# caskcsg/lightretriever

Hardware: AMD Instinct MI355X
Metric: docs embedded/sec (llama3.2-1b dims, seq_len=512, bf16) [+ queries/sec@top-100 over 1000000-doc index in `search`] (higher is better)
Workload: dtype bf16

## Files before the change

include/lrx.h:

```cpp
#ifndef LRX_H
#define LRX_H

#include <stddef.h>
#include <stdint.h>

#ifdef __cplusplus
extern "C" {
#endif

#define LRX_ABI_VERSION 8

enum {
  LRX_OK = 0,
  LRX_ERR_INVALID = -1,
  LRX_ERR_HIP = -2,
  LRX_ERR_WORKSPACE = -3,
};

int lrx_abi_version(void);
const char* lrx_last_error(void);

typedef struct lrx_encoder_config {
  int32_t vocab_size;
  int32_t hidden_size;
// ... 125 lines not shown
                       int32_t capacity, int32_t* ids_out, int32_t* weights_out, int32_t* counts_out, void* stream);

int lrx_sparse_csr_count(const float* reps, int32_t n_rows, int32_t vocab_size, int64_t row_stride, int32_t quantization_factor,
                         int32_t empty_marker, int32_t* counts_out, void* stream);
int lrx_sparse_csr_fill(const float* reps, int32_t n_rows, int32_t vocab_size, int64_t row_stride, int32_t quantization_factor,
                        int32_t empty_marker, const int64_t* row_off, int32_t* terms_out, int32_t* weights_out, void* stream);

int lrx_hit_contributions(const double* scores, const int64_t* ids, int32_t n_queries, int32_t k, int64_t row_stride,
                          int32_t method, double param0, double param1, double* contrib_out, int64_t contrib_row_stride,
                          void* stream);
int lrx_hit_union(const int64_t* ids, const double* contrib, int32_t n_queries, int32_t n_entries, int64_t row_stride,
                  double* scores_out, int64_t* ids_out, int32_t* counts_out, void* stream);

int lrx_gemm_bf16_nt_fused(const void* A, const void* B, void* C, const void* bias, const void* resid, int32_t M, int32_t N,
                           int32_t K, int32_t epilogue, const float* rscale, float* ss_part, void* stream);
int lrx_gemm_qkv_rope_fused(const void* A, const void* Wqkv, void* C, const void* bias, const int32_t* positions,
                            const float* cos, const float* sin, int32_t M, int32_t K, int32_t num_q_heads,
                            int32_t num_kv_heads, int32_t head_dim, const float* rscale, void* stream);
int lrx_gemm_qkv_rope_slice(const void* A, const void* Wqkv, void* C, const void* bias, const int32_t* positions,
                            const float* cos, const float* sin, int32_t M, int32_t K, int32_t num_q_heads,
                            int32_t num_kv_heads, int32_t head_dim, const float* rscale, int32_t head0, int32_t n_heads, void* stream);
int lrx_gemm_bf16_nt_resid32(const void* A, const void* B, float* x32, void* a16_out, const void* gamma, int32_t M, int32_t N,
                             int32_t K, float* ss_part, void* stream);
int lrx_embed_stream32(const void* table, const int32_t* ids, int32_t n_tokens, int32_t hidden, int32_t vocab, const void* gamma,
                       float* x32, void* a16, float* rscale_out, float eps, void* stream);
int lrx_rmsnorm_f32(const float* x, const void* w, void* y, int32_t rows, int32_t hidden, float eps, void* stream);
int lrx_row_rscale(const void* x, int32_t rows, int32_t hidden_size, float eps, float* rscale_out, void* stream);
int lrx_finalize_rscale(const float* ss_part, int32_t n_parts, int32_t rows, int32_t hidden_size, float eps, float* rscale_out,
                        void* stream);

int lrx_gather_last_rows(const void* src, const int32_t* cu_seqlens, int32_t n_seqs, int32_t width, void* dst, void* stream);
int lrx_scatter_last_rows(const void* src, const int32_t* cu_seqlens, int32_t n_seqs, int32_t width, void* dst, int64_t dst_row_stride,
                          void* stream);

int lrx_pool_norm(const void* hidden, const void* final_norm_w, const int32_t* cu_seqlens, int32_t n_seqs,
                  int32_t hidden_size, float eps, float* out, int64_t out_row_stride, int32_t out_dim,
                  int32_t normalize, void* stream);
int lrx_pool_norm_shard(const void* hidden, const void* final_norm_w, const int32_t* cu_seqlens, int32_t n_seqs,
                        int32_t hidden_size, float eps, float* out, int64_t out_row_stride, int32_t out_dim,
                        int32_t normalize, void* shadow_out, int64_t shadow_row0, float* row_bounds, int32_t hidden_f32, void* stream);

int lrx_pool_norm_mode(const void* hidden, const void* final_norm_w, const int32_t* cu_seqlens, int32_t n_seqs,
                       int32_t hidden_size, float eps, int32_t pooling, float* out, int64_t out_row_stride, int32_t out_dim,
                       int32_t normalize, void* shadow_out, int64_t shadow_row0, float* row_bounds, int32_t hidden_f32, void* stream);

int lrx_embedding_bag_mean(const float* table, int32_t vocab, int32_t hidden, const int64_t* ids, int64_t n_ids,
// ... 129 lines not shown
```

lightretriever_amd/_lib.py:

```python
import ctypes as C
import os

HERE = os.path.dirname(os.path.abspath(__file__))
LIB_PATH = os.environ.get("LRX_LIB_DEV_VARIANT") or os.path.join(HERE, "liblrx.so")
LRX_PROF_CLASSES = 8
ABI_VERSION = 8
SEARCH_FILTER_AUTO, SEARCH_FILTER_MATRIX, SEARCH_FILTER_SCORE_FREE, SEARCH_FILTER_SCORE_FREE_NO_GEMM = 0, 1, 2, 3
SEARCH_FUSED_ALWAYS, SEARCH_FUSED_NEVER = 4, 8
SEARCH_REFINE_ROWS_ALWAYS, SEARCH_REFINE_ROWS_NEVER = 16, 32
BINARY_SELECT_ONLY = 1
PROF_CLASS_NAMES = ["gemm_store", "gemm_resid", "gemm_swiglu", "attention", "rmsnorm", "rope", "other", "gemm_maxagg"]


class LrxError(RuntimeError):
    pass


class EncoderConfigC(C.Structure):
    _fields_ = [("vocab_size", C.c_int32), ("hidden_size", C.c_int32), ("num_layers", C.c_int32), ("num_q_heads", C.c_int32),
                ("num_kv_heads", C.c_int32), ("head_dim", C.c_int32), ("intermediate_size", C.c_int32), ("rms_eps", C.c_float),
                ("qkv_bias", C.c_int32), ("max_positions", C.c_int32), ("norm_folded", C.c_int32), ("precise_stream", C.c_int32)]


class LayerWeightsC(C.Structure):
# ... 60 lines not shown
    "lrx_pq_ip_search": (_I32, [_P, _I64, _P, _I32, _I32, _P, _I32, _I32, _I64, _P, _P, _P, _P, _SZ, _I32, _P]),
    "lrx_pq_encode": (_I32, [_P, _I64, _I64, _P, _I32, _I32, _P, _I64, _P]),
    "lrx_pq_decode_rows": (_I32, [_P, _I64, _I64, _P, _I32, _I32, _P, _I64, _P]),
    "lrx_pq_lut": (_I32, [_P, _I32, _P, _I32, _I32, _P, _P]),
    "lrx_binary_workspace_bytes": (_SZ, [_I64, _I32, _I32, _I32]),
    "lrx_binary_hamming_search": (_I32, [_P, _I64, _I32, _P, _I32, _F, _P, _I32, _I64, _P, _P, _P, _P, _SZ, _I32, _P]),
    "lrx_binary_ip_search": (_I32, [_P, _I64, _I32, _P, _I32, _F, _P, _I32, _I32, _I64, _P, _P, _P, _P, _SZ, _I32, _P]),
    "lrx_binary_pack_rows": (_I32, [_P, _I64, _I64, _I32, _F, _P, _P, _I64, _P]),
    "lrx_binary_store_rows": (_I32, [_P, _I64, _I64, _I32, _P, _I64, _P]),
    "lrx_binary_decode_rows": (_I32, [_P, _I64, _I64, _I32, _P, _I64, _P]),
    "lrx_sq8_ip_workspace_bytes": (_SZ, [_I64, _I32, _I32, _I32]),
    "lrx_sq8_ip_chunk_queries": (_I32, [_I64, _I32, _I32, _I32]),
    "lrx_sq8_ip_search": (_I32, [_P, _I64, _P, _I32, _I32, _P, _I32, _I32, _I64, _P, _P, _P, _P, _SZ, _I32, _P]),
    "lrx_sq8_train_minmax": (_I32, [_P, _I64, _I64, _I32, _P, _P]),
    "lrx_sq8_encode": (_I32, [_P, _I64, _I64, _P, _I32, _I32, _P, _I64, _P]),
    "lrx_sq8_decode_rows": (_I32, [_P, _I64, _I64, _P, _I32, _I32, _P, _I64, _P]),
    "lrx_linear_transform": (_I32, [_P, _I64, _I64, _P, _P, _I32, _I32, _P, _I64, _P]),
    "lrx_impact_workspace_bytes": (_SZ, [_I64, _I32, _I32]),
    "lrx_impact_chunk_queries": (_I32, [_I64, _I32, _I32]),
    "lrx_impact_search": (_I32, [_P, _P, _I32, _I64, _P, _P, _P, _I32, _I32, _I64, _P, _P, _P, _P, _SZ, _I32, _P]),
    "lrx_shard_commit_rows": (_I32, [_P, _I64, _I64, _I32, _P, _I64, _P, _P]),
    "lrx_pool_norm_shard": (_I32, [_P, _P, _P, _I32, _I32, _F, _P, _I64, _I32, _I32, _P, _I64, _P, _I32, _P]),
    "lrx_gemm_bf16_nt_resid32": (_I32, [_P, _P, _P, _P, _P, _I32, _I32, _I32, _P, _P]),
    "lrx_embed_stream32": (_I32, [_P, _P, _I32, _I32, _I32, _P, _P, _P, _P, _F, _P]),
    "lrx_rmsnorm_f32": (_I32, [_P, _P, _P, _I32, _I32, _F, _P]),
    "lrx_gemm_bf16_nt_fused": (_I32, [_P, _P, _P, _P, _P, _I32, _I32, _I32, _I32, _P, _P, _P]),
    "lrx_gemm_qkv_rope_fused": (_I32, [_P, _P, _P, _P, _P, _P, _P, _I32, _I32, _I32, _I32, _I32, _P, _P]),
    "lrx_row_rscale": (_I32, [_P, _I32, _I32, C.c_float, _P, _P]),
    "lrx_finalize_rscale": (_I32, [_P, _I32, _I32, _I32, C.c_float, _P, _P]),
    "lrx_set_profiling": (None, [_I32]),
    "lrx_get_profile": (_I32, [C.POINTER(C.c_float), C.POINTER(C.c_double), C.POINTER(C.c_int32)]),
    "lrx_embedding_gather": (_I32, [_P, _P, _I32, _I32, _I32, _P, _P]),
    "lrx_trace_marker": (_I32, [_I32, _P]),
    "lrx_probe_stream_read": (_I32, [_P, _SZ, _P, _I32, _P]),
    "lrx_device_error_count": (_I64, [_I32]),
    "lrx_device_saturation_count": (_I64, [_I32]),
    "lrx_rmsnorm": (_I32, [_P, _P, _P, _I32, _I32, _F, _P]),
    "lrx_gemm_bf16_nt": (_I32, [_P, _P, _P, _P, _P, _I32, _I32, _I32, _I32, _P]),
    "lrx_gemm_qkv_rope": (_I32, [_P, _P, _P, _P, _P, _P, _P, _I32, _I32, _I32, _I32, _I32, _P]),
    "lrx_build_positions": (_I32, [_P, _I32, _I32, _P, _P]),
    "lrx_attn_varlen_causal": (_I32, [_P, _P, _I32, _I32, _I32, _I32, _I32, _I32, _P, _I32, _P]),
    "lrx_attn_items_bytes": (_SZ, [_I32, _I32, _I32, _I32, _I32, _I32, _I32]),
    "lrx_attn_build_items": (_I32, [_P, _I32, _I32, _I32, _I32, _I32, _I32, _I32, _P, _SZ, _P]),
    "lrx_attn_varlen_causal_items": (_I32, [_P, _P, _P, _SZ, _I32, _I32, _I32, _I32, _I32, _I32, _P, _I32, _P]),
    "lrx_debug_attn_items_overflow": (_I32, [_P]),
    "lrx_gather_last_rows": (_I32, [_P, _P, _I32, _I32, _P, _P]),
# ... 55 lines not shown
```

lightretriever_amd/csrc/lrx_gemm.hip:

```cpp
#include "lrx_common.h"
#include <float.h>
#include <stdlib.h>

#define GBM 256
#define GBN 256
#define GBK 64
#define HALF_BYTES 16384

enum { EPI_STORE = 0, EPI_RESID = 1, EPI_SWIGLU = 2, EPI_ROPE = 3, EPI_MAXAGG = 4, EPI_EMIT = 5, EPI_RESID32 = 6, EPI_SAMPLE = 7 };
#define EPI_IS_SEARCH(E) ((E) == EPI_EMIT || (E) == EPI_SAMPLE)

struct RopeArgs {
  const int32_t* positions;
  const float* cos;
  const float* sin;
  int rope_cols;
  int head_dim;
  int ldc;
};

__device__ __forceinline__ __bf16 f2h_bits(float v) {
  return __builtin_bit_cast(__bf16, (_Float16)fminf(fmaxf(v, -65504.f), 65504.f));
}
__device__ unsigned int g_qkv_fp16_saturations = 0;
// ... 39 lines not shown

typedef const __attribute__((address_space(1))) void* gptr_t;
typedef __attribute__((address_space(3))) void* lptr_t;

#define G_BAR()                            \
  do {                                     \
    __builtin_amdgcn_sched_barrier(0);     \
    __builtin_amdgcn_s_barrier();          \
    __builtin_amdgcn_sched_barrier(0);     \
  } while (0)
#define G_LSYNC()                                          \
  do {                                                     \
    asm volatile("s_waitcnt lgkmcnt(0)" ::: "memory");     \
    G_BAR();                                               \
  } while (0)



typedef __attribute__((ext_vector_type(8))) _Float16 f16x8;
template <int EPI, bool F16>
__device__ __forceinline__ f32x4 gemm_mfma(bf16x8 x, bf16x8 y, f32x4 c) {
  if constexpr (EPI_IS_SEARCH(EPI) || F16) return __builtin_amdgcn_mfma_f32_16x16x32_f16(__builtin_bit_cast(f16x8, x), __builtin_bit_cast(f16x8, y), c, 0, 0, 0);
  else return __builtin_amdgcn_mfma_f32_16x16x32_bf16(x, y, c, 0, 0, 0);
}

template <int EPI, bool F16 = false, bool OUTH = F16>
__global__ void __launch_bounds__(512, 2)
k_gemm_bf16_nt(const __bf16* __restrict__ A, const __bf16* __restrict__ B, __bf16* C, const __bf16* __restrict__ bias,
               const __bf16* resid, int M, int N, int K, int tiles_m, int tiles_n, RopeArgs rope, MaxAggArgs mx, NormArgs nrm, EmitArgs em) {
  __shared__ __attribute__((aligned(1024))) char smem[8 * HALF_BYTES + (EPI == EPI_EMIT ? 2304 : 0)];
  const int nwg = gridDim.x, bid = blockIdx.x;
  const int xcd = bid & 7, qd = nwg >> 3, rm = nwg & 7;
  const int t_lin = (xcd < rm ? xcd * (qd + 1) : rm * (qd + 1) + (xcd - rm) * qd) + (bid >> 3);
  const int GM = nrm.group_m;
  const int width = GM * tiles_n;
  const int group = t_lin / width, first_m = group * GM;
  const int gsz = min(tiles_m - first_m, GM);
  const int tin = t_lin - group * width;
  const int tm = first_m + tin % gsz, tn = tin / gsz;
  const int tmx = EPI == EPI_SAMPLE ? tm * em.ss : ((EPI == EPI_EMIT && em.ss > 1) ? (tm / (em.ss - 1)) * em.ss + 1 + tm % (em.ss - 1) : tm);
  const int m0 = tmx * GBM, n0 = tn * GBN;

  const int tid = threadIdx.x, lane = tid & 63;
  const int wave = __builtin_amdgcn_readfirstlane(tid >> 6);
  const int wr = wave >> 2, wc = wave & 3;
  if constexpr (EPI == EPI_EMIT) {
// ... 199 lines not shown
                    const unsigned int gp = atomicAdd(&em.cnt[(n0 + col) * CNT_STRIDE], 1u);
                    if (gp < em.cap) em.cand[(int64_t)(n0 + col) * em.cap + gp] = w;
                  }
                  ++p;
                }
            }
          }
      }
    __syncthreads();
    if (tid < GBN) {
      const unsigned int n = qc[tid];
      if (n) qc[tid] = atomicAdd(&em.cnt[(n0 + tid) * CNT_STRIDE], n);
    }
    __syncthreads();
    const unsigned int total = min(*wn, (unsigned int)WCAP);
    for (unsigned int i = lane; i < total; i += 64) {
      const unsigned long long w = wl[i];
      const unsigned int e = wq[i], col = e & 255u;
      const unsigned int gp = qc[col] + (e >> 8);
      if (gp < em.cap) em.cand[(int64_t)(n0 + col) * em.cap + gp] = w;
    }
    return;
  }
  if constexpr (EPI == EPI_RESID32) {
    float* x32 = (float*)resid;
    const int nq4 = n0 + lane * 4;
    const bool nin = nq4 < N;
    float gm[4] = {1.f, 1.f, 1.f, 1.f};
    if (bias != nullptr && nin) {
      const bf16x4 g4 = *(const bf16x4*)(bias + nq4);
#pragma unroll
      for (int e = 0; e < 4; ++e) gm[e] = bf2f(g4[e]);
    }
#pragma unroll
    for (int p = 0; p < 2; ++p) {
      f32x4 rv[16];
#pragma unroll
      for (int it = 0; it < 16; ++it) {
        const int m = m0 + p * 128 + it * 8 + wave;
        rv[it] = (m < M && nin) ? *(const f32x4*)(x32 + (int64_t)m * N + nq4) : f32x4{0.f, 0.f, 0.f, 0.f};
      }
      if (p) __syncthreads();
#pragma unroll
      for (int hp = 0; hp < 2; ++hp)
#pragma unroll
        for (int mi = 0; mi < 4; ++mi)
#pragma unroll
          for (int ni = 0; ni < 2; ++ni) {
            const int row = wr * 64 + mi * 16 + fr, chunk = hp * 32 + wc * 8 + ni * 4 + fq;
            *(f32x4*)(smem + row * 1024 + ((chunk ^ ((row & 15) << 2)) << 4)) = acc[p][hp][mi][ni];
          }
      __syncthreads();
#pragma unroll
      for (int it = 0; it < 16; ++it) {
        const int row = it * 8 + wave, m = m0 + p * 128 + row;
        f32x4 v = *(const f32x4*)(smem + row * 1024 + ((lane ^ ((row & 15) << 2)) << 4));
        const bool inb = m < M && nin;
#pragma unroll
        for (int e = 0; e < 4; ++e) v[e] += rv[it][e];
        if (inb) {
          *(f32x4*)(x32 + (int64_t)m * N + nq4) = v;
          if (C != nullptr) {
            bf16x4 a4;
            if constexpr (OUTH) {
              bool sat = false;
#pragma unroll
              for (int e = 0; e < 4; ++e) { const float t = v[e] * gm[e]; sat |= !(fabsf(t) <= 65504.f); a4[e] = f2h_bits(t); }
              if (__any(sat)) { if ((int)(threadIdx.x & 63) == __ffsll((long long)__ballot(1)) - 1) atomicAdd(&g_qkv_fp16_saturations, 1u); }
            } else {
#pragma unroll
              for (int e = 0; e < 4; ++e) a4[e] = f2bf(v[e] * gm[e]);
            }
            *(bf16x4*)(C + (int64_t)m * N + nq4) = a4;
          }
        }
        if (nrm.ss_part != nullptr) {
          float ssq = inb ? (v[0] * v[0] + v[1] * v[1]) + (v[2] * v[2] + v[3] * v[3]) : 0.f;
          ssq += __int_as_float(__builtin_amdgcn_update_dpp(0, __float_as_int(ssq), 0x128, 0xF, 0xF, true));
          ssq += __int_as_float(__builtin_amdgcn_update_dpp(0, __float_as_int(ssq), 0x124, 0xF, 0xF, true));
          ssq += __int_as_float(__builtin_amdgcn_update_dpp(0, __float_as_int(ssq), 0x4E, 0xF, 0xF, true));
          ssq += __int_as_float(__builtin_amdgcn_update_dpp(0, __float_as_int(ssq), 0xB1, 0xF, 0xF, true));
          ssq += __int_as_float(__builtin_amdgcn_update_dpp(0, __float_as_int(ssq), 0x142, 0xA, 0xF, false));
          ssq += __int_as_float(__builtin_amdgcn_update_dpp(0, __float_as_int(ssq), 0x143, 0xC, 0xF, false));
          if (lane == 63 && m < M) nrm.ss_part[(int64_t)tn * M + m] = ssq;
        }
      }
    }
    return;
  }
  constexpr int CW = (EPI == EPI_SWIGLU) ? 128 : 256;
  constexpr int CPR = CW / 8;
  constexpr int NIT = (256 * CPR) / 512;
  bf16x8 rv[EPI == EPI_RESID ? NIT : 1];
  if (EPI == EPI_RESID) {
    const int ldc_ = N, c0_ = n0;
#pragma unroll
    for (int it = 0; it < NIT; ++it) {
      const int q = it * 512 + tid;
      const int m = min(m0 + q / CPR, M - 1), n = min(c0_ + (q % CPR) * 8, ldc_ - 8);
      rv[it] = *(const bf16x8*)(resid + (int64_t)m * N + n);
    }
  }
#pragma unroll
  for (int h = 0; h < 2; ++h)
#pragma unroll
    for (int mi = 0; mi < 4; ++mi) {
      const int row = h * 128 + wr * 64 + mi * 16 + fr;
      const float rs = rsv[h][mi];
#pragma unroll
      for (int hp = 0; hp < 2; ++hp) {
        if (EPI == EPI_SWIGLU) {
          bf16x4 o;
          bool sat = false;
#pragma unroll
          for (int r = 0; r < 4; ++r) {
            const float g = acc[h][hp][mi][0][r] * rs, u = acc[h][hp][mi][1][r] * rs;
            const float sg = __builtin_amdgcn_rcpf(1.0f + __builtin_amdgcn_exp2f(g * -1.4426950408889634f));
            const float t = g * sg * u;
            if constexpr (F16) { sat |= !(fabsf(t) <= 65504.f); o[r] = f2h_bits(t); }
            else o[r] = f2bf(t);
          }
          if constexpr (F16) { if (__any(sat)) { if ((int)(threadIdx.x & 63) == __ffsll((long long)__ballot(1)) - 1) atomicAdd(&g_qkv_fp16_saturations, 1u); } }
          const int col = hp * 64 + wc * 16 + fq * 4;
          *(bf16x4*)(smem + row * (CW * 2) + ((((col >> 3) ^ (row & 15)) << 4) | ((col & 4) << 1))) = o;
        } else if (EPI == EPI_ROPE) {
          const int cb = hp * 128 + wc * 32;
          const bool rot = n0 + cb < rope.rope_cols;
          f32x4 x1 = acc[h][hp][mi][0], x2 = acc[h][hp][mi][1];
#pragma unroll
          for (int r = 0; r < 4; ++r) { x1[r] *= rs; x2[r] *= rs; }
          if (bias != nullptr) {
            const int nb = min(n0 + cb + fq * 4, N - 20);
            const bf16x4 b1 = *(const bf16x4*)(bias + nb), b2 = *(const bf16x4*)(bias + nb + 16);
#pragma unroll
            for (int r = 0; r < 4; ++r) { x1[r] += bf2f(b1[r]); x2[r] += bf2f(b2[r]); }
          }
          if (rot) {
            const int rhalf = rope.head_dim >> 1;
            const int j = (((n0 + cb) % rope.head_dim) >> 5) * 16 + fq * 4;
            const f32x4 cc = *(const f32x4*)(rope.cos + (int64_t)rposv[h][mi] * rhalf + j), sn = *(const f32x4*)(rope.sin + (int64_t)rposv[h][mi] * rhalf + j);
#pragma unroll
            for (int r = 0; r < 4; ++r) {
              const float a = x1[r], b = x2[r];
              x1[r] = a * cc[r] - b * sn[r];
              x2[r] = b * cc[r] + a * sn[r];
            }
          }
          bf16x4 o1, o2;
          bool sat = false;
#pragma unroll
          for (int r = 0; r < 4; ++r) {
            sat |= !(fabsf(x1[r]) <= 65504.f) | !(fabsf(x2[r]) <= 65504.f);
            o1[r] = f2h_bits(x1[r]);
            o2[r] = f2h_bits(x2[r]);
          }
          if (__any(sat)) { if ((int)(threadIdx.x & 63) == __ffsll((long long)__ballot(1)) - 1) atomicAdd(&g_qkv_fp16_saturations, 1u); }
          const int c1 = cb + fq * 4, c2 = c1 + 16;
          *(bf16x4*)(smem + row * (CW * 2) + ((((c1 >> 3) ^ (row & 15)) << 4) | ((c1 & 4) << 1))) = o1;
          *(bf16x4*)(smem + row * (CW * 2) + ((((c2 >> 3) ^ (row & 15)) << 4) | ((c2 & 4) << 1))) = o2;
        } else {
#pragma unroll
          for (int ni = 0; ni < 2; ++ni) {
            const int col = hp * 128 + wc * 32 + ni * 16 + fq * 4;
            f32x4 v = acc[h][hp][mi][ni];
            if (EPI == EPI_STORE) {
#pragma unroll
              for (int r = 0; r < 4; ++r) v[r] *= rs;
            }
            if (EPI == EPI_STORE && bias != nullptr) {
              const int n = min(n0 + col, N - 4);
              bf16x4 bv = *(const bf16x4*)(bias + n);
#pragma unroll
              for (int r = 0; r < 4; ++r) v[r] += bf2f(bv[r]);
            }
            if (EPI == EPI_MAXAGG && bias != nullptr) {
#pragma unroll
              for (int r = 0; r < 4; ++r) v[r] += bf2f(bias[min(n0 + col + r, N - 1)]);
            }
            bf16x4 o;
#pragma unroll
            for (int r = 0; r < 4; ++r) o[r] = f2bf(v[r]);
            *(bf16x4*)(smem + row * (CW * 2) + ((((col >> 3) ^ (row & 15)) << 4) | ((col & 4) << 1))) = o;
          }
        }
      }
    }
  __syncthreads();
  if (EPI == EPI_MAXAGG) {
    const int colq = wave * 32 + (lane & 7) * 4;
    const int choff = colq >> 3, hb = (colq & 4) << 1;
    const float NEG = -__builtin_inff();
    float m4[4] = {NEG, NEG, NEG, NEG};
    int cur = -1;
    auto flush = [&](int seg) {
      if (seg < 0) return;
#pragma unroll
      for (int r = 0; r < 4; ++r)
        if (n0 + colq + r < N && m4[r] != NEG) atomic_fmax_bits(mx.out + (int64_t)seg * mx.ldo + n0 + colq + r, m4[r]);
    };
    for (int step = 0; step < 32; ++step) {
      const int row = step * 8 + (lane >> 3);
      const int m = m0 + row;
      const int seg = m < M ? mx.row_seg[m] : -1;
      if (seg >= 0) {
        if (seg != cur) {
          flush(cur);
          cur = seg;
#pragma unroll
          for (int r = 0; r < 4; ++r) m4[r] = NEG;
// ... 3 lines not shown
        for (int r = 0; r < 4; ++r) m4[r] = fmaxf(m4[r], bf2f(v[r]));
      }
    }
    int cmax = cur;
#pragma unroll
    for (int o = 32; o >= 1; o >>= 1) cmax = max(cmax, __shfl_xor(cmax, o));
    const bool uniform = __all(cur == cmax || cur == -1);
    if (uniform) {
      if (cur == -1) {
#pragma unroll
        for (int r = 0; r < 4; ++r) m4[r] = NEG;
      }
#pragma unroll
      for (int o = 8; o <= 32; o <<= 1)
#pragma unroll
        for (int r = 0; r < 4; ++r) m4[r] = fmaxf(m4[r], __shfl_xor(m4[r], o));
      if ((lane >> 3) == 0) flush(cmax);
    } else {
      flush(cur);
    }
    return;
  }
  const int ncols = (EPI == EPI_SWIGLU) ? (N >> 1) : N;
  const int ldc = (EPI == EPI_ROPE && rope.ldc > 0) ? rope.ldc : ncols;
  const int c0 = (EPI == EPI_SWIGLU) ? (n0 >> 1) : n0;
  {
#pragma unroll
  for (int it = 0; it < NIT; ++it) {
    const int q = it * 512 + tid;
    const int row = q / CPR, ch = q % CPR;
    const int m = m0 + row, n = c0 + ch * 8;
    const bool inb = m < M && n < ncols;
    if (!(EPI == EPI_RESID && nrm.ss_part != nullptr) && !inb) continue;
    bf16x8 v = *(const bf16x8*)(smem + row * (CW * 2) + ((ch ^ (row & 15)) << 4));
    if (EPI == EPI_RESID) {
#pragma unroll
      for (int e = 0; e < 8; ++e) v[e] = f2bf(bf2f(v[e]) + bf2f(rv[it][e]));
      if (nrm.ss_part != nullptr) {
        float ssq = 0.f;
#pragma unroll
        for (int e = 0; e < 8; ++e) { const float f = bf2f(v[e]); ssq += f * f; }
        if (!inb) ssq = 0.f;
        ssq += __int_as_float(__builtin_amdgcn_update_dpp(0, __float_as_int(ssq), 0x128, 0xF, 0xF, true));
        ssq += __int_as_float(__builtin_amdgcn_update_dpp(0, __float_as_int(ssq), 0x124, 0xF, 0xF, true));
        ssq += __int_as_float(__builtin_amdgcn_update_dpp(0, __float_as_int(ssq), 0x4E, 0xF, 0xF, true));
        ssq += __int_as_float(__builtin_amdgcn_update_dpp(0, __float_as_int(ssq), 0xB1, 0xF, 0xF, true));
        ssq += __shfl_xor(ssq, 16, 64);
// ... 85 lines not shown
  const int N = n_heads * head_dim, col0 = head0 * head_dim;
  const int rope_cols = (num_q_heads + num_kv_heads) * head_dim - col0;
  int tiles_m = (int)lrx_cdiv(M, GBM), tiles_n = (int)lrx_cdiv(N, GBN);
  RopeArgs rope = {positions, cos, sin, rope_cols < 0 ? 0 : (rope_cols > N ? N : rope_cols), head_dim, n_all * head_dim};
  if (f16)
    hipLaunchKernelGGL((k_gemm_bf16_nt<EPI_ROPE, true>), dim3(tiles_m * tiles_n), dim3(512), 0, (hipStream_t)stream, (const __bf16*)A,
                       (const __bf16*)Wqkv + (int64_t)col0 * K, (__bf16*)C + col0, bias ? (const __bf16*)bias + col0 : (const __bf16*)nullptr,
                       (const __bf16*)nullptr, M, N, K, tiles_m, tiles_n, rope, MaxAggArgs{nullptr, nullptr, 0}, NormArgs{rscale, nullptr, 8},
                       EmitArgs{nullptr, nullptr, nullptr, 0, 0u, nullptr, nullptr, 0, 0});
  else
  hipLaunchKernelGGL(k_gemm_bf16_nt<EPI_ROPE>, dim3(tiles_m * tiles_n), dim3(512), 0, (hipStream_t)stream, (const __bf16*)A,
                     (const __bf16*)Wqkv + (int64_t)col0 * K, (__bf16*)C + col0, bias ? (const __bf16*)bias + col0 : (const __bf16*)nullptr,
                     (const __bf16*)nullptr, M, N, K, tiles_m, tiles_n, rope, MaxAggArgs{nullptr, nullptr, 0}, NormArgs{rscale, nullptr, 8},
                     EmitArgs{nullptr, nullptr, nullptr, 0, 0u, nullptr, nullptr, 0, 0});
  LRX_LAUNCH_CHECK();
  return LRX_OK;
}

extern "C" int lrx_gemm_bf16_nt_resid32(const void* A, const void* B, float* x32, void* a16_out, const void* gamma, int32_t M, int32_t N, int32_t K,
                                        float* ss_part, void* stream) {
  return lrx_gemm_nt_resid32_ex(A, B, x32, a16_out, gamma, M, N, K, ss_part, 0, 0, stream);
}

int lrx_gemm_nt_resid32_ex(const void* A, const void* B, float* x32, void* a16_out, const void* gamma, int32_t M, int32_t N, int32_t K, float* ss_part,
                           int f16, int out_f16, void* stream) {
  LRX_CHECK_ARG(!f16 || out_f16 || a16_out == nullptr, "gemm_resid32: fp16 operands write an fp16 operand");
  LRX_CHECK_ARG(M >= 0 && N > 0 && K > 0 && K % GBK == 0 && N % 8 == 0, "gemm_resid32: bad shape M=%d N=%d K=%d", M, N, K);
  LRX_CHECK_ARG(x32 != nullptr, "gemm_resid32: null residual stream");
  if (M == 0) return LRX_OK;
  int tiles_m = (int)lrx_cdiv(M, GBM), tiles_n = (int)lrx_cdiv(N, GBN);
  RopeArgs none = {nullptr, nullptr, nullptr, 0, 64, 0};
  if (f16)
    hipLaunchKernelGGL((k_gemm_bf16_nt<EPI_RESID32, true>), dim3(tiles_m * tiles_n), dim3(512), 0, (hipStream_t)stream, (const __bf16*)A, (const __bf16*)B,
                       (__bf16*)a16_out, (const __bf16*)gamma, (const __bf16*)x32, M, N, K, tiles_m, tiles_n, none, MaxAggArgs{nullptr, nullptr, 0},
                       NormArgs{nullptr, ss_part, gemm_group_m(EPI_RESID, K)}, EmitArgs{nullptr, nullptr, nullptr, 0, 0u, nullptr, nullptr, 0, 0});
  else if (out_f16 && a16_out != nullptr)
    hipLaunchKernelGGL((k_gemm_bf16_nt<EPI_RESID32, false, true>), dim3(tiles_m * tiles_n), dim3(512), 0, (hipStream_t)stream, (const __bf16*)A, (const __bf16*)B,
                       (__bf16*)a16_out, (const __bf16*)gamma, (const __bf16*)x32, M, N, K, tiles_m, tiles_n, none, MaxAggArgs{nullptr, nullptr, 0},
                       NormArgs{nullptr, ss_part, gemm_group_m(EPI_RESID, K)}, EmitArgs{nullptr, nullptr, nullptr, 0, 0u, nullptr, nullptr, 0, 0});
  else
  hipLaunchKernelGGL(k_gemm_bf16_nt<EPI_RESID32>, dim3(tiles_m * tiles_n), dim3(512), 0, (hipStream_t)stream, (const __bf16*)A, (const __bf16*)B,
                     (__bf16*)a16_out, (const __bf16*)gamma, (const __bf16*)x32, M, N, K, tiles_m, tiles_n, none, MaxAggArgs{nullptr, nullptr, 0},
                     NormArgs{nullptr, ss_part, gemm_group_m(EPI_RESID, K)}, EmitArgs{nullptr, nullptr, nullptr, 0, 0u, nullptr, nullptr, 0, 0});
  LRX_LAUNCH_CHECK();
  return LRX_OK;
}
// ... 51 lines not shown
```

lightretriever_amd/ops.py:

```python
from __future__ import annotations

from typing import Optional

import torch

from . import _lib


def _s():
    return _lib.current_stream()


def embedding_gather(table: torch.Tensor, ids: torch.Tensor) -> torch.Tensor:
    out = torch.empty(ids.numel(), table.shape[1], dtype=torch.bfloat16, device=table.device)
    _lib.check(_lib.lib().lrx_embedding_gather(_lib.ptr(table), _lib.ptr(ids), ids.numel(), table.shape[1], table.shape[0], _lib.ptr(out), _s()))
    return out


def rmsnorm(x: torch.Tensor, w: torch.Tensor, eps: float) -> torch.Tensor:
    y = torch.empty_like(x)
    _lib.check(_lib.lib().lrx_rmsnorm(_lib.ptr(x), _lib.ptr(w), _lib.ptr(y), x.shape[0], x.shape[1], eps, _s()))
    return y


# ... 39 lines not shown
    return torch.cat([rot, torch.arange((nq + nkv) * d, (nq + 2 * nkv) * d)])


def gemm_qkv_rope(A: torch.Tensor, Wqkv: torch.Tensor, positions: torch.Tensor, cos: torch.Tensor, sin: torch.Tensor, nq: int, nkv: int,
                  d: int, bias: Optional[torch.Tensor] = None, rscale: Optional[torch.Tensor] = None) -> torch.Tensor:
    M, K = A.shape
    out = torch.empty(M, (nq + 2 * nkv) * d, dtype=torch.float16, device=A.device)
    _lib.check(_lib.lib().lrx_gemm_qkv_rope_fused(_lib.ptr(A), _lib.ptr(Wqkv), _lib.ptr(out), _lib.ptr(bias), _lib.ptr(positions), _lib.ptr(cos),
                                                  _lib.ptr(sin), M, K, nq, nkv, d, _lib.ptr(rscale), _s()))
    return out


def gemm_qkv_rope_slice(A: torch.Tensor, Wqkv: torch.Tensor, positions: torch.Tensor, cos: torch.Tensor, sin: torch.Tensor, nq: int, nkv: int,
                        d: int, head0: int, n_heads: int, out: torch.Tensor, bias: Optional[torch.Tensor] = None,
                        rscale: Optional[torch.Tensor] = None) -> torch.Tensor:
    M, K = A.shape
    if out.dtype != torch.float16 or out.shape != (M, (nq + 2 * nkv) * d) or not out.is_contiguous():
        raise ValueError("gemm_qkv_rope_slice: out must be contiguous fp16 [M, (nq+2nkv)d]")
    _lib.check(_lib.lib().lrx_gemm_qkv_rope_slice(_lib.ptr(A), _lib.ptr(Wqkv), _lib.ptr(out), _lib.ptr(bias), _lib.ptr(positions), _lib.ptr(cos),
                                                  _lib.ptr(sin), M, K, nq, nkv, d, _lib.ptr(rscale), head0, n_heads, _s()))
    return out


def gemm_resid32(A: torch.Tensor, B: torch.Tensor, x32: torch.Tensor, gamma: Optional[torch.Tensor] = None, want_a16: bool = True, want_ss: bool = False):
    M, K = A.shape
    N = B.shape[0]
    a16 = torch.empty(M, N, dtype=torch.bfloat16, device=A.device) if want_a16 else None
    ss = torch.full(((N + 255) // 256, M), float("nan"), dtype=torch.float32, device=A.device) if want_ss else None
    _lib.check(_lib.lib().lrx_gemm_bf16_nt_resid32(_lib.ptr(A), _lib.ptr(B), _lib.ptr(x32), _lib.ptr(a16), _lib.ptr(gamma), M, N, K, _lib.ptr(ss), _s()))
    return a16, ss


def embed_stream32(table: torch.Tensor, ids: torch.Tensor, gamma: torch.Tensor, eps: float):
    T, H = ids.numel(), table.shape[1]
    x32 = torch.empty(T, H, dtype=torch.float32, device=table.device)
    a16 = torch.empty(T, H, dtype=torch.bfloat16, device=table.device)
    rs = torch.empty(T, dtype=torch.float32, device=table.device)
    _lib.check(_lib.lib().lrx_embed_stream32(_lib.ptr(table), _lib.ptr(ids), T, H, table.shape[0], _lib.ptr(gamma), _lib.ptr(x32), _lib.ptr(a16), _lib.ptr(rs),
                                             float(eps), _s()))
    return x32, a16, rs


def rmsnorm_f32(x: torch.Tensor, w: torch.Tensor, eps: float) -> torch.Tensor:
    y = torch.empty(x.shape, dtype=torch.bfloat16, device=x.device)
    _lib.check(_lib.lib().lrx_rmsnorm_f32(_lib.ptr(x), _lib.ptr(w), _lib.ptr(y), x.shape[0], x.shape[1], float(eps), _s()))
    return y


def build_positions(cu_seqlens: torch.Tensor, total_tokens: int) -> torch.Tensor:
    pos = torch.empty(total_tokens, dtype=torch.int32, device=cu_seqlens.device)
    _lib.check(_lib.lib().lrx_build_positions(_lib.ptr(cu_seqlens), cu_seqlens.numel() - 1, total_tokens, _lib.ptr(pos), _s()))
    return pos
# ... 144 lines not shown
```

Measured before the change: 1348.

## Specialize resid32 and RoPE GEMM epilogues for full tiles with pipelined smem reads

Moves the resid32 and RoPE epilogues into separate templated functions with full-tile fast paths. These paths drop the per-row bounds checks, prefetch the next group of shared-memory rows and the cos/sin table entries ahead of use, and hoist the fp16 saturation ballot out of the inner loops. The goal is lower epilogue instruction count and latency in the encoder GEMMs. It also adds an f16-output resid32 entry point, and it slightly changes floating-point contraction behaviour (explicit fma use), which may alter rounding.

```diff
diff --git a/include/lrx.h b/include/lrx.h
--- a/include/lrx.h
+++ b/include/lrx.h
@@ -171,6 +171,8 @@
                             int32_t num_kv_heads, int32_t head_dim, const float* rscale, int32_t head0, int32_t n_heads, void* stream);
 int lrx_gemm_bf16_nt_resid32(const void* A, const void* B, float* x32, void* a16_out, const void* gamma, int32_t M, int32_t N,
                              int32_t K, float* ss_part, void* stream);
+int lrx_gemm_bf16_nt_resid32_f16out(const void* A, const void* B, float* x32, void* a16_out, const void* gamma, int32_t M, int32_t N,
+                                    int32_t K, float* ss_part, void* stream);
 int lrx_embed_stream32(const void* table, const int32_t* ids, int32_t n_tokens, int32_t hidden, int32_t vocab, const void* gamma,
                        float* x32, void* a16, float* rscale_out, float eps, void* stream);
 int lrx_rmsnorm_f32(const float* x, const void* w, void* y, int32_t rows, int32_t hidden, float eps, void* stream);
diff --git a/lightretriever_amd/_lib.py b/lightretriever_amd/_lib.py
--- a/lightretriever_amd/_lib.py
+++ b/lightretriever_amd/_lib.py
@@ -106,6 +106,7 @@
     "lrx_shard_commit_rows": (_I32, [_P, _I64, _I64, _I32, _P, _I64, _P, _P]),
     "lrx_pool_norm_shard": (_I32, [_P, _P, _P, _I32, _I32, _F, _P, _I64, _I32, _I32, _P, _I64, _P, _I32, _P]),
     "lrx_gemm_bf16_nt_resid32": (_I32, [_P, _P, _P, _P, _P, _I32, _I32, _I32, _P, _P]),
+    "lrx_gemm_bf16_nt_resid32_f16out": (_I32, [_P, _P, _P, _P, _P, _I32, _I32, _I32, _P, _P]),
     "lrx_embed_stream32": (_I32, [_P, _P, _I32, _I32, _I32, _P, _P, _P, _P, _F, _P]),
     "lrx_rmsnorm_f32": (_I32, [_P, _P, _P, _I32, _I32, _F, _P]),
     "lrx_gemm_bf16_nt_fused": (_I32, [_P, _P, _P, _P, _P, _I32, _I32, _I32, _I32, _P, _P, _P]),
diff --git a/lightretriever_amd/csrc/lrx_gemm.hip b/lightretriever_amd/csrc/lrx_gemm.hip
--- a/lightretriever_amd/csrc/lrx_gemm.hip
+++ b/lightretriever_amd/csrc/lrx_gemm.hip
@@ -85,6 +85,226 @@
 __device__ __forceinline__ f32x4 gemm_mfma(bf16x8 x, bf16x8 y, f32x4 c) {
   if constexpr (EPI_IS_SEARCH(EPI) || F16) return __builtin_amdgcn_mfma_f32_16x16x32_f16(__builtin_bit_cast(f16x8, x), __builtin_bit_cast(f16x8, y), c, 0, 0, 0);
   else return __builtin_amdgcn_mfma_f32_16x16x32_bf16(x, y, c, 0, 0, 0);
+}
+
+__device__ __forceinline__ void report_fp16_saturation(bool sat) {
+  if (__any(sat)) { if ((int)(threadIdx.x & 63) == __ffsll((long long)__ballot(1)) - 1) atomicAdd(&g_qkv_fp16_saturations, 1u); }
+}
+
+template <bool FMA>
+__device__ __forceinline__ float sum_sq4(const f32x4 v) {
+#pragma clang fp contract(off)
+  if constexpr (FMA) return __builtin_fmaf(v[0], v[0], v[1] * v[1]) + __builtin_fmaf(v[2], v[2], v[3] * v[3]);
+  else return (v[0] * v[0] + v[1] * v[1]) + (v[2] * v[2] + v[3] * v[3]);
+}
+__device__ __forceinline__ void rotate4(f32x4& x1, f32x4& x2, const f32x4 cc, const f32x4 sn) {
+#pragma clang fp contract(off)
+#pragma unroll
+  for (int r = 0; r < 4; ++r) {
+    const float a = x1[r], b = x2[r];
+    if (r < 2) { x1[r] = __builtin_fmaf(a, cc[r], -(b * sn[r])); x2[r] = __builtin_fmaf(b, cc[r], a * sn[r]); }
+    else { x1[r] = a * cc[r] - b * sn[r]; x2[r] = b * cc[r] + a * sn[r]; }
+  }
+}
+__device__ __forceinline__ f32x4 scale4(const f32x4 x, float s) {
+#pragma clang fp contract(off)
+  return f32x4{x[0] * s, x[1] * s, x[2] * s, x[3] * s};
+}
+
+#ifdef LRX_GEMM_FULL_TILES_ONLY
+#define G_TILE_IS_FULL(COND) true
+#else
+#define G_TILE_IS_FULL(COND) __builtin_expect((COND), 1)
+#endif
+
+template <bool FULL, bool OUTH, bool NEXT>
+__device__ __forceinline__ void gemm_resid32_epilogue(char* smem, const f32x4 (&acc)[2][2][4][2], float* x32, __bf16* C, const __bf16* gamma, float* ss_part,
+                                                      int M, int N, int m0, int n0, int tn, int wave, int lane, int wr, int wc, int fr, int fq) {
+  const bool next = FULL ? NEXT : C != nullptr;
+  const bool want_ss = FULL ? NEXT : ss_part != nullptr;
+  const int nq4 = n0 + lane * 4;
+  const bool nin = FULL || nq4 < N;
+  float gm[4] = {1.f, 1.f, 1.f, 1.f};
+  if (gamma != nullptr && nin) {
+    const bf16x4 g4 = *(const bf16x4*)(gamma + nq4);
+#pragma unroll
+    for (int e = 0; e < 4; ++e) gm[e] = bf2f(g4[e]);
+  }
+  const int64_t tile0 = (int64_t)(m0 + wave) * N + n0;
+  const size_t xstep = (size_t)N * 32, cstep = (size_t)N * 16;
+  const unsigned xlane = (unsigned)lane * 16u, clane = (unsigned)lane * 8u;
+  bool sat = false;
+#pragma unroll
+  for (int p = 0; p < 2; ++p) {
+    char* const xrow = (char*)(x32 + tile0) + (size_t)p * 16 * xstep;
+    char* const crow = (char*)(C + tile0) + (size_t)p * 16 * cstep;
+    f32x4 rv[16];
+    {
+      const char* q = xrow;
+#pragma unroll
+      for (int it = 0; it < 16; ++it, q += xstep)
+        rv[it] = (FULL || (m0 + p * 128 + it * 8 + wave < M && nin)) ? *(const f32x4*)(q + xlane) : f32x4{0.f, 0.f, 0.f, 0.f};
+    }
+    if (p) __syncthreads();
+#pragma unroll
+    for (int hp = 0; hp < 2; ++hp)
+#pragma unroll
+      for (int mi = 0; mi < 4; ++mi)
+#pragma unroll
+        for (int ni = 0; ni < 2; ++ni) {
+          const int row = wr * 64 + mi * 16 + fr, chunk = hp * 32 + wc * 8 + ni * 4 + fq;
+          *(f32x4*)(smem + row * 1024 + ((chunk ^ ((row & 15) << 2)) << 4)) = acc[p][hp][mi][ni];
+        }
+    __syncthreads();
+    float ssv = 0.f;
+    f32x4 nx[4];
+#define G_R32_READ(G)                                                                                      \
+  _Pragma("unroll") for (int r = 0; r < 4; ++r) {                                                          \
+    const int row = ((G) * 4 + r) * 8 + wave;                                                              \
+    nx[r] = *(const f32x4*)(smem + row * 1024 + ((lane ^ ((row & 15) << 2)) << 4));                        \
+  }
+    G_R32_READ(0)
+    char* xq = xrow;
+    char* cq = crow;
+#pragma unroll
+    for (int g = 0; g < 4; ++g) {
+      f32x4 v[4];
+      bool inb[4];
+#pragma unroll
+      for (int r = 0; r < 4; ++r) {
+        v[r] = nx[r];
+        inb[r] = FULL || (m0 + p * 128 + (g * 4 + r) * 8 + wave < M && nin);
+      }
+      if (g < 3) G_R32_READ(g + 1)
+#pragma unroll
+      for (int r = 0; r < 4; ++r) {
+#pragma unroll
+        for (int e = 0; e < 4; ++e) v[r][e] += rv[g * 4 + r][e];
+        if (inb[r]) *(f32x4*)(xq + r * xstep + xlane) = v[r];
+      }
+      if (next) {
+#pragma unroll
+        for (int r = 0; r < 4; ++r) {
+          bf16x4 a4;
+          if constexpr (OUTH) {
+#pragma unroll
+            for (int e = 0; e < 4; ++e) { const float t = v[r][e] * gm[e]; sat |= inb[r] && !(fabsf(t) <= 65504.f); a4[e] = f2h_bits(t); }
+          } else {
+#pragma unroll
+            for (int e = 0; e < 4; ++e) a4[e] = f2bf(v[r][e] * gm[e]);
+          }
+          if (inb[r]) *(bf16x4*)(cq + r * cstep + clane) = a4;
+        }
+      }
+      if (want_ss) {
+        float ssq[4];
+#pragma unroll
+        for (int r = 0; r < 4; ++r) ssq[r] = inb[r] ? sum_sq4<OUTH>(v[r]) : 0.f;
+#define G_R32_DPP(CTRL, ROWMASK, BOUND)                                                                                                      \
+  _Pragma("unroll") for (int r = 0; r < 4; ++r) ssq[r] += __int_as_float(__builtin_amdgcn_update_dpp(0, __float_as_int(ssq[r]), CTRL, ROWMASK, 0xF, BOUND));
+        G_R32_DPP(0x128, 0xF, true)
+        G_R32_DPP(0x124, 0xF, true)
+        G_R32_DPP(0x4E, 0xF, true)
+        G_R32_DPP(0xB1, 0xF, true)
+        G_R32_DPP(0x142, 0xA, false)
+        G_R32_DPP(0x143, 0xC, false)
+#undef G_R32_DPP
+#pragma unroll
+        for (int r = 0; r < 4; ++r) {
+          int tot = __builtin_amdgcn_readlane(__float_as_int(ssq[r]), 63);
+          asm volatile("" : "+s"(tot));
+          ssv = lane == g * 4 + r ? __int_as_float(tot) : ssv;
+        }
+      }
+      xq += 4 * xstep;
+      cq += 4 * cstep;
+    }
+#undef G_R32_READ
+    if (want_ss) {
+      const int m = m0 + p * 128 + lane * 8 + wave;
+      if (lane < 16 && (FULL || m < M)) ss_part[(int64_t)tn * M + m] = ssv;
+    }
+  }
+  if constexpr (OUTH) report_fp16_saturation(sat);
+}
+
+template <bool FULL>
+__device__ __forceinline__ void gemm_rope_epilogue(char* smem, const f32x4 (&acc)[2][2][4][2], __bf16* C, const __bf16* bias, const RopeArgs& rope,
+                                                   const float (&rsv)[2][4], const int (&rposv)[2][4], int M, int N, int m0, int n0, int tid, int wr, int wc,
+                                                   int fr, int fq) {
+  const int rhalf = rope.head_dim >> 1;
+  bool rot[2];
+  int jc[2];
+#pragma unroll
+  for (int hp = 0; hp < 2; ++hp) {
+    const int cb = hp * 128 + wc * 32;
+    rot[hp] = FULL || n0 + cb < rope.rope_cols;
+    jc[hp] = (((n0 + cb) & (rope.head_dim - 1)) >> 5) * 16 + fq * 4;
+  }
+  unsigned satm = 0u;
+  f32x4 ccn[2], snn[2];
+#define G_ROPE_TABLE(H, MI)                                                                                    \
+  _Pragma("unroll") for (int hp = 0; hp < 2; ++hp) {                                                           \
+    const int64_t t = (int64_t)rposv[H][MI] * rhalf + jc[hp];                                                  \
+    ccn[hp] = *(const f32x4*)(rope.cos + t);                                                                   \
+    snn[hp] = *(const f32x4*)(rope.sin + t);                                                                   \
+  }
+  if constexpr (FULL) { G_ROPE_TABLE(0, 0) }
+#pragma unroll
+  for (int h = 0; h < 2; ++h)
+#pragma unroll
+    for (int mi = 0; mi < 4; ++mi) {
+      const int row = h * 128 + wr * 64 + mi * 16 + fr;
+      const float rs = rsv[h][mi];
+      const int64_t trow = (int64_t)rposv[h][mi] * rhalf;
+      f32x4 ccv[2], snv[2];
+      if constexpr (FULL) {
+#pragma unroll
+        for (int hp = 0; hp < 2; ++hp) { ccv[hp] = ccn[hp]; snv[hp] = snn[hp]; }
+        if (h * 4 + mi < 7) { G_ROPE_TABLE((h * 4 + mi + 1) >> 2, (h * 4 + mi + 1) & 3) }
+      }
+#pragma unroll
+      for (int hp = 0; hp < 2; ++hp) {
+        const int cb = hp * 128 + wc * 32;
+        f32x4 x1 = scale4(acc[h][hp][mi][0], rs), x2 = scale4(acc[h][hp][mi][1], rs);
+        if (!FULL && bias != nullptr) {
+          const int nb = min(n0 + cb + fq * 4, N - 20);
+          const bf16x4 b1 = *(const bf16x4*)(bias + nb), b2 = *(const bf16x4*)(bias + nb + 16);
+#pragma unroll
+          for (int r = 0; r < 4; ++r) { x1[r] += bf2f(b1[r]); x2[r] += bf2f(b2[r]); }
+        }
+        if (rot[hp]) {
+          f32x4 cc, sn;
+          if constexpr (FULL) { cc = ccv[hp]; sn = snv[hp]; }
+          else { cc = *(const f32x4*)(rope.cos + trow + jc[hp]); sn = *(const f32x4*)(rope.sin + trow + jc[hp]); }
+          rotate4(x1, x2, cc, sn);
+        }
+        bf16x4 o1, o2;
+#pragma unroll
+        for (int r = 0; r < 4; ++r) {
+          satm = max(satm, max(__float_as_uint(x1[r]) & 0x7fffffffu, __float_as_uint(x2[r]) & 0x7fffffffu));
+          o1[r] = f2h_bits(x1[r]);
+          o2[r] = f2h_bits(x2[r]);
+        }
+        const int c1 = cb + fq * 4, c2 = c1 + 16;
+        *(bf16x4*)(smem + row * 512 + ((((c1 >> 3) ^ (row & 15)) << 4) | ((c1 & 4) << 1))) = o1;
+        *(bf16x4*)(smem + row * 512 + ((((c2 >> 3) ^ (row & 15)) << 4) | ((c2 & 4) << 1))) = o2;
+      }
+      __builtin_amdgcn_sched_barrier(0);
+    }
+#undef G_ROPE_TABLE
+  report_fp16_saturation(satm > 0x477fe000u);
+  __syncthreads();
+  const int ldc = rope.ldc > 0 ? rope.ldc : N;
+  const int r0 = tid >> 5, ch = tid & 31;
+  const char* lp = smem + r0 * 512 + ((ch ^ (r0 & 15)) << 4);
+  char* cp = (char*)(C + ((int64_t)(m0 + r0) * ldc + n0 + ch * 8));
+  const size_t cstep = (size_t)ldc * 32;
+#pragma unroll
+  for (int it = 0; it < 16; ++it, cp += cstep) {
+    if (!FULL && !(m0 + it * 16 + r0 < M && n0 + ch * 8 < N)) continue;
+    *(bf16x8*)cp = *(const bf16x8*)(lp + it * 8192);
+  }
 }
 
 template <int EPI, bool F16 = false, bool OUTH = F16>
@@ -330,69 +550,26 @@
     }
     return;
   }
+  if constexpr (EPI == EPI_ROPE) {
+    if (G_TILE_IS_FULL(m0 + GBM <= M && n0 + GBN <= N && n0 + GBN <= rope.rope_cols && bias == nullptr)) {
+      gemm_rope_epilogue<true>(smem, acc, C, bias, rope, rsv, rposv, M, N, m0, n0, tid, wr, wc, fr, fq);
+    } else {
+      gemm_rope_epilogue<false>(smem, acc, C, bias, rope, rsv, rposv, M, N, m0, n0, tid, wr, wc, fr, fq);
+    }
+    return;
+  }
   if constexpr (EPI == EPI_RESID32) {
     float* x32 = (float*)resid;
-    const int nq4 = n0 + lane * 4;
-    const bool nin = nq4 < N;
-    float gm[4] = {1.f, 1.f, 1.f, 1.f};
-    if (bias != nullptr && nin) {
-      const bf16x4 g4 = *(const bf16x4*)(bias + nq4);
-#pragma unroll
-      for (int e = 0; e < 4; ++e) gm[e] = bf2f(g4[e]);
-    }
-#pragma unroll
-    for (int p = 0; p < 2; ++p) {
-      f32x4 rv[16];
-#pragma unroll
-      for (int it = 0; it < 16; ++it) {
-        const int m = m0 + p * 128 + it * 8 + wave;
-        rv[it] = (m < M && nin) ? *(const f32x4*)(x32 + (int64_t)m * N + nq4) : f32x4{0.f, 0.f, 0.f, 0.f};
-      }
-      if (p) __syncthreads();
-#pragma unroll
-      for (int hp = 0; hp < 2; ++hp)
-#pragma unroll
-        for (int mi = 0; mi < 4; ++mi)
-#pragma unroll
-          for (int ni = 0; ni < 2; ++ni) {
-            const int row = wr * 64 + mi * 16 + fr, chunk = hp * 32 + wc * 8 + ni * 4 + fq;
-            *(f32x4*)(smem + row * 1024 + ((chunk ^ ((row & 15) << 2)) << 4)) = acc[p][hp][mi][ni];
-          }
-      __syncthreads();
-#pragma unroll
-      for (int it = 0; it < 16; ++it) {
-        const int row = it * 8 + wave, m = m0 + p * 128 + row;
-        f32x4 v = *(const f32x4*)(smem + row * 1024 + ((lane ^ ((row & 15) << 2)) << 4));
-        const bool inb = m < M && nin;
-#pragma unroll
-        for (int e = 0; e < 4; ++e) v[e] += rv[it][e];
-        if (inb) {
-          *(f32x4*)(x32 + (int64_t)m * N + nq4) = v;
-          if (C != nullptr) {
-            bf16x4 a4;
-            if constexpr (OUTH) {
-              bool sat = false;
-#pragma unroll
-              for (int e = 0; e < 4; ++e) { const float t = v[e] * gm[e]; sat |= !(fabsf(t) <= 65504.f); a4[e] = f2h_bits(t); }
-              if (__any(sat)) { if ((int)(threadIdx.x & 63) == __ffsll((long long)__ballot(1)) - 1) atomicAdd(&g_qkv_fp16_saturations, 1u); }
-            } else {
-#pragma unroll
-              for (int e = 0; e < 4; ++e) a4[e] = f2bf(v[e] * gm[e]);
-            }
-            *(bf16x4*)(C + (int64_t)m * N + nq4) = a4;
-          }
-        }
-        if (nrm.ss_part != nullptr) {
-          float ssq = inb ? (v[0] * v[0] + v[1] * v[1]) + (v[2] * v[2] + v[3] * v[3]) : 0.f;
-          ssq += __int_as_float(__builtin_amdgcn_update_dpp(0, __float_as_int(ssq), 0x128, 0xF, 0xF, true));
-          ssq += __int_as_float(__builtin_amdgcn_update_dpp(0, __float_as_int(ssq), 0x124, 0xF, 0xF, true));
-          ssq += __int_as_float(__builtin_amdgcn_update_dpp(0, __float_as_int(ssq), 0x4E, 0xF, 0xF, true));
-          ssq += __int_as_float(__builtin_amdgcn_update_dpp(0, __float_as_int(ssq), 0xB1, 0xF, 0xF, true));
-          ssq += __int_as_float(__builtin_amdgcn_update_dpp(0, __float_as_int(ssq), 0x142, 0xA, 0xF, false));
-          ssq += __int_as_float(__builtin_amdgcn_update_dpp(0, __float_as_int(ssq), 0x143, 0xC, 0xF, false));
-          if (lane == 63 && m < M) nrm.ss_part[(int64_t)tn * M + m] = ssq;
-        }
-      }
+#ifdef LRX_GEMM_FULL_TILES_ONLY
+    const bool both = true, neither = false;
+#else
+    const bool both = C != nullptr && nrm.ss_part != nullptr, neither = C == nullptr && nrm.ss_part == nullptr;
+#endif
+    if (G_TILE_IS_FULL(m0 + GBM <= M && n0 + GBN <= N && (both || neither))) {
+      if (both) gemm_resid32_epilogue<true, OUTH, true>(smem, acc, x32, C, bias, nrm.ss_part, M, N, m0, n0, tn, wave, lane, wr, wc, fr, fq);
+      else gemm_resid32_epilogue<true, OUTH, false>(smem, acc, x32, C, bias, nrm.ss_part, M, N, m0, n0, tn, wave, lane, wr, wc, fr, fq);
+    } else {
+      gemm_resid32_epilogue<false, OUTH, false>(smem, acc, x32, C, bias, nrm.ss_part, M, N, m0, n0, tn, wave, lane, wr, wc, fr, fq);
     }
     return;
   }
@@ -409,6 +586,7 @@
       rv[it] = *(const bf16x8*)(resid + (int64_t)m * N + n);
     }
   }
+  bool sat = false;
 #pragma unroll
   for (int h = 0; h < 2; ++h)
 #pragma unroll
@@ -419,7 +597,6 @@
       for (int hp = 0; hp < 2; ++hp) {
         if (EPI == EPI_SWIGLU) {
           bf16x4 o;
-          bool sat = false;
 #pragma unroll
           for (int r = 0; r < 4; ++r) {
             const float g = acc[h][hp][mi][0][r] * rs, u = acc[h][hp][mi][1][r] * rs;
@@ -428,44 +605,8 @@
             if constexpr (F16) { sat |= !(fabsf(t) <= 65504.f); o[r] = f2h_bits(t); }
             else o[r] = f2bf(t);
           }
-          if constexpr (F16) { if (__any(sat)) { if ((int)(threadIdx.x & 63) == __ffsll((long long)__ballot(1)) - 1) atomicAdd(&g_qkv_fp16_saturations, 1u); } }
           const int col = hp * 64 + wc * 16 + fq * 4;
           *(bf16x4*)(smem + row * (CW * 2) + ((((col >> 3) ^ (row & 15)) << 4) | ((col & 4) << 1))) = o;
-        } else if (EPI == EPI_ROPE) {
-          const int cb = hp * 128 + wc * 32;
-          const bool rot = n0 + cb < rope.rope_cols;
-          f32x4 x1 = acc[h][hp][mi][0], x2 = acc[h][hp][mi][1];
-#pragma unroll
-          for (int r = 0; r < 4; ++r) { x1[r] *= rs; x2[r] *= rs; }
-          if (bias != nullptr) {
-            const int nb = min(n0 + cb + fq * 4, N - 20);
-            const bf16x4 b1 = *(const bf16x4*)(bias + nb), b2 = *(const bf16x4*)(bias + nb + 16);
-#pragma unroll
-            for (int r = 0; r < 4; ++r) { x1[r] += bf2f(b1[r]); x2[r] += bf2f(b2[r]); }
-          }
-          if (rot) {
-            const int rhalf = rope.head_dim >> 1;
-            const int j = (((n0 + cb) % rope.head_dim) >> 5) * 16 + fq * 4;
-            const f32x4 cc = *(const f32x4*)(rope.cos + (int64_t)rposv[h][mi] * rhalf + j), sn = *(const f32x4*)(rope.sin + (int64_t)rposv[h][mi] * rhalf + j);
-#pragma unroll
-            for (int r = 0; r < 4; ++r) {
-              const float a = x1[r], b = x2[r];
-              x1[r] = a * cc[r] - b * sn[r];
-              x2[r] = b * cc[r] + a * sn[r];
-            }
-          }
-          bf16x4 o1, o2;
-          bool sat = false;
-#pragma unroll
-          for (int r = 0; r < 4; ++r) {
-            sat |= !(fabsf(x1[r]) <= 65504.f) | !(fabsf(x2[r]) <= 65504.f);
-            o1[r] = f2h_bits(x1[r]);
-            o2[r] = f2h_bits(x2[r]);
-          }
-          if (__any(sat)) { if ((int)(threadIdx.x & 63) == __ffsll((long long)__ballot(1)) - 1) atomicAdd(&g_qkv_fp16_saturations, 1u); }
-          const int c1 = cb + fq * 4, c2 = c1 + 16;
-          *(bf16x4*)(smem + row * (CW * 2) + ((((c1 >> 3) ^ (row & 15)) << 4) | ((c1 & 4) << 1))) = o1;
-          *(bf16x4*)(smem + row * (CW * 2) + ((((c2 >> 3) ^ (row & 15)) << 4) | ((c2 & 4) << 1))) = o2;
         } else {
 #pragma unroll
           for (int ni = 0; ni < 2; ++ni) {
@@ -493,6 +634,7 @@
         }
       }
     }
+  if constexpr (EPI == EPI_SWIGLU && F16) report_fp16_saturation(sat);
   __syncthreads();
   if (EPI == EPI_MAXAGG) {
     const int colq = wave * 32 + (lane & 7) * 4;
@@ -542,7 +684,7 @@
     return;
   }
   const int ncols = (EPI == EPI_SWIGLU) ? (N >> 1) : N;
-  const int ldc = (EPI == EPI_ROPE && rope.ldc > 0) ? rope.ldc : ncols;
+  const int ldc = ncols;
   const int c0 = (EPI == EPI_SWIGLU) ? (n0 >> 1) : n0;
   {
 #pragma unroll
@@ -674,6 +816,11 @@
   return lrx_gemm_nt_resid32_ex(A, B, x32, a16_out, gamma, M, N, K, ss_part, 0, 0, stream);
 }
 
+extern "C" int lrx_gemm_bf16_nt_resid32_f16out(const void* A, const void* B, float* x32, void* a16_out, const void* gamma, int32_t M, int32_t N, int32_t K,
+                                               float* ss_part, void* stream) {
+  return lrx_gemm_nt_resid32_ex(A, B, x32, a16_out, gamma, M, N, K, ss_part, 0, 1, stream);
+}
+
 int lrx_gemm_nt_resid32_ex(const void* A, const void* B, float* x32, void* a16_out, const void* gamma, int32_t M, int32_t N, int32_t K, float* ss_part,
                            int f16, int out_f16, void* stream) {
   LRX_CHECK_ARG(!f16 || out_f16 || a16_out == nullptr, "gemm_resid32: fp16 operands write an fp16 operand");
diff --git a/lightretriever_amd/ops.py b/lightretriever_amd/ops.py
--- a/lightretriever_amd/ops.py
+++ b/lightretriever_amd/ops.py
@@ -85,12 +85,14 @@
     return out
 
 
-def gemm_resid32(A: torch.Tensor, B: torch.Tensor, x32: torch.Tensor, gamma: Optional[torch.Tensor] = None, want_a16: bool = True, want_ss: bool = False):
+def gemm_resid32(A: torch.Tensor, B: torch.Tensor, x32: torch.Tensor, gamma: Optional[torch.Tensor] = None, want_a16: bool = True, want_ss: bool = False,
+                 out_f16: bool = False):
     M, K = A.shape
     N = B.shape[0]
-    a16 = torch.empty(M, N, dtype=torch.bfloat16, device=A.device) if want_a16 else None
+    a16 = torch.empty(M, N, dtype=torch.float16 if out_f16 else torch.bfloat16, device=A.device) if want_a16 else None
     ss = torch.full(((N + 255) // 256, M), float("nan"), dtype=torch.float32, device=A.device) if want_ss else None
-    _lib.check(_lib.lib().lrx_gemm_bf16_nt_resid32(_lib.ptr(A), _lib.ptr(B), _lib.ptr(x32), _lib.ptr(a16), _lib.ptr(gamma), M, N, K, _lib.ptr(ss), _s()))
+    fn = _lib.lib().lrx_gemm_bf16_nt_resid32_f16out if out_f16 else _lib.lib().lrx_gemm_bf16_nt_resid32
+    _lib.check(fn(_lib.ptr(A), _lib.ptr(B), _lib.ptr(x32), _lib.ptr(a16), _lib.ptr(gamma), M, N, K, _lib.ptr(ss), _s()))
     return a16, ss
 
 
```

New measurement: 1354, median of 6. No clear change (+0.5%).
